# DuckTapeDevOps/kubernetes-cloud

Measured on AMD Instinct MI355X. Metric: GPT-J-6B finetune tokens/sec, higher is better.
Workload: dtype bf16; 1 GPU; model=gpt-j-6b, global_batch=32, micro_batch=16, grad_accum=2, seq_len=2048, parallelism=dp1, activation_checkpointing=False

## Files before the change

csrc/kernels/attention_tiled.hip:

```cpp
#include "common.h"

#include <type_traits>

namespace {

constexpr float kLog2e = 1.4426950408889634f;
constexpr float kLn2 = 0.6931471805599453f;
constexpr float kRescaleThr = 8.0f;

#ifdef KCA_ATTN_STAMPS
__device__ unsigned long long g_attn_stamps[64];
__device__ __forceinline__ unsigned long long ast_now() {
  unsigned long long t;
  __builtin_amdgcn_sched_barrier(0);
  asm volatile("s_memtime %0\n\ts_waitcnt lgkmcnt(0)" : "=s"(t)::"memory");
  __builtin_amdgcn_sched_barrier(0);
  return t;
}
#define ASTAMP_DECL                                            \
  unsigned long long st_acc_[8] = {0, 0, 0, 0, 0, 0, 0, 0}; \
  unsigned long long st_prev_ = ast_now();
#define ASTAMP(k)                           \
  do {                                      \
    const unsigned long long n_ = ast_now(); \
    st_acc_[k] += n_ - st_prev_;            \
    st_prev_ = n_;                          \
  } while (0)
#define ASTAMP_FLUSH(base)                                                          \
  do {                                                                              \
    st_acc_[7] = 1;                                                                 \
    if ((threadIdx.x & 63) == 0)                                                    \
      for (int i_ = 0; i_ < 8; ++i_) atomicAdd(&g_attn_stamps[(base) + i_], st_acc_[i_]); \
  } while (0)
#else
#define ASTAMP_DECL
#define ASTAMP(k) \
  do {            \
  } while (0)
#define ASTAMP_FLUSH(base) \
  do {                     \
  } while (0)
#endif


struct FastFwdParams {
  const bf16_t* q; const bf16_t* k; const bf16_t* v;
  bf16_t* o; float* lse;
  int* flags;
  long long q_sb, q_st, q_sh, k_sb, k_st, k_sh, v_sb, v_st, v_sh;
  long long o_sb, o_st, o_sh;
  int B, Sq, Sk, H, Hkv;
  float scale;
};

typedef __attribute__((address_space(3))) bf16x4 lds_bf16x4_t;
typedef unsigned int u32x4 __attribute__((ext_vector_type(4)));

__device__ __forceinline__ bf16x4 lds_tr4(const char* base, int byte_off) {
  return __builtin_amdgcn_ds_read_tr16_b64_v4bf16(
      (lds_bf16x4_t*)(reinterpret_cast<uintptr_t>(base + byte_off)));
}

__device__ __forceinline__ bf16x8 lds_b128(const char* base, int byte_off) {
  return *reinterpret_cast<const bf16x8*>(base + byte_off);
}

template <int D>
__device__ __forceinline__ int img_off(int row, int ch) {
  return (row >> 3) * 16 * D + 512 * (ch >> 2) + 64 * (row & 7) + 16 * ((ch & 3) ^ ((row >> 2) & 3));
}

__device__ __forceinline__ bf16x8 cat8(bf16x4 a, bf16x4 b) {
  return __builtin_shufflevector(a, b, 0, 1, 2, 3, 4, 5, 6, 7);
}

__device__ __forceinline__ uint32_t pk_bf16(float lo, float hi) {
  return pack_bf16x2(lo, hi);
}

__device__ __forceinline__ __amdgpu_buffer_rsrc_t head_rsrc(const bf16_t* b) {
  const unsigned long long a = (unsigned long long)b;
  const unsigned long long au = ((unsigned long long)__builtin_amdgcn_readfirstlane((unsigned)(a >> 32)) << 32) |
                                (unsigned)__builtin_amdgcn_readfirstlane((unsigned)a);
  return __builtin_amdgcn_make_buffer_rsrc((void*)au, (short)0, 0x7fffffff, 0x00020000);
}

template <int D, bool POW2 = (256 % (D / 8)) == 0>
struct Stager;

template <int D>
struct Stager<D, true> {
  static constexpr int NCH = D / 8, CPT = 32 * NCH / 256, RPI = 256 / NCH;
  long long ok_, ov_;
  int row0_, ch_;
  __amdgpu_buffer_rsrc_t rk_, rv_;
  int vok_[CPT], vov_[CPT];
  __device__ __forceinline__ Stager(int tid, long long k_st, long long v_st) {
    row0_ = tid / NCH;
    ch_ = tid % NCH;
    ok_ = (long long)row0_ * k_st + ch_ * 8;
    ov_ = (long long)row0_ * v_st + ch_ * 8;
  }
  __device__ __forceinline__ void bind(const bf16_t* kb, const bf16_t* vb, long long k_st, long long v_st) {
#pragma unroll
    for (int i = 0; i < CPT; ++i) {
      vok_[i] = (int)((ok_ + (long long)i * RPI * k_st) * 2);
      vov_[i] = (int)((ov_ + (long long)i * RPI * v_st) * 2);
    }
    set_base(kb, vb);
  }
  __device__ __forceinline__ void set_base(const bf16_t* kb, const bf16_t* vb) {
    rk_ = head_rsrc(kb);
    rv_ = head_rsrc(vb);
  }
  __device__ __forceinline__ void load(u32x4 (&sk)[CPT], u32x4 (&sv)[CPT], const bf16_t* kb, const bf16_t* vb,
                                       int k0, long long k_st, long long v_st) const {
    const int sok = __builtin_amdgcn_readfirstlane((int)(k0 * k_st * 2));
    const int sov = __builtin_amdgcn_readfirstlane((int)(k0 * v_st * 2));
#pragma unroll
    for (int i = 0; i < CPT; ++i) {
      const auto a = __builtin_amdgcn_raw_buffer_load_b128(rk_, vok_[i], sok, 0);
      const auto b = __builtin_amdgcn_raw_buffer_load_b128(rv_, vov_[i], sov, 0);
      sk[i] = *reinterpret_cast<const u32x4*>(&a);
      sv[i] = *reinterpret_cast<const u32x4*>(&b);
    }
  }
  __device__ __forceinline__ void store(const u32x4 (&sk)[CPT], const u32x4 (&sv)[CPT], char* buf) const {
#pragma unroll
    for (int i = 0; i < CPT; ++i) {
      const int o = img_off<D>(row0_ + i * RPI, ch_);
      *reinterpret_cast<u32x4*>(buf + o) = sk[i];
      *reinterpret_cast<u32x4*>(buf + 32 * D * 2 + o) = sv[i];
    }
  }
};

template <int D>
struct Stager<D, false> {
  static constexpr int NCH = D / 8, TOT = 32 * NCH, CPT = (TOT + 255) / 256;
  static_assert(D % 32 == 0 && TOT % 64 == 0, "tiled attention: D multiple of 32");
  long long ok_[CPT], ov_[CPT];
  int lds_[CPT];
  bool tail_;
  __device__ __forceinline__ Stager(int tid, long long k_st, long long v_st) {
#pragma unroll
    for (int i = 0; i < CPT; ++i) {
      const int idx = min(tid + 256 * i, TOT - 1);
      const int row = idx / NCH, ch = idx % NCH;
      ok_[i] = (long long)row * k_st + ch * 8;
      ov_[i] = (long long)row * v_st + ch * 8;
      lds_[i] = img_off<D>(row, ch);
    }
    tail_ = tid + 256 * (CPT - 1) < TOT;
  }
  __device__ __forceinline__ void bind(const bf16_t*, const bf16_t*, long long, long long) {}
  __device__ __forceinline__ void set_base(const bf16_t*, const bf16_t*) {}
  __device__ __forceinline__ void load(u32x4 (&sk)[CPT], u32x4 (&sv)[CPT], const bf16_t* kb, const bf16_t* vb,
                                       int k0, long long k_st, long long v_st) const {
    const bf16_t* kr = kb + (long long)k0 * k_st;
    const bf16_t* vr = vb + (long long)k0 * v_st;
#pragma unroll
    for (int i = 0; i < CPT; ++i) {
      sk[i] = *reinterpret_cast<const u32x4*>(kr + ok_[i]);
      sv[i] = *reinterpret_cast<const u32x4*>(vr + ov_[i]);
    }
  }
  __device__ __forceinline__ void store(const u32x4 (&sk)[CPT], const u32x4 (&sv)[CPT], char* buf) const {
#pragma unroll
    for (int i = 0; i < CPT; ++i) {
      if (i < CPT - 1 || tail_) {
        *reinterpret_cast<u32x4*>(buf + lds_[i]) = sk[i];
        *reinterpret_cast<u32x4*>(buf + 32 * D * 2 + lds_[i]) = sv[i];
      }
    }
  }
};

template <int D, int DS>
struct StagerNarrow {
  static constexpr int NCH = DS / 8, TOT = 32 * NCH, CPT = 1;
  static_assert(TOT <= 256 && TOT % 64 == 0, "narrow stager: one chunk per thread, whole waves");
  int vok_[1], vov_[1], lds_;
  bool on_;
  __amdgpu_buffer_rsrc_t rk_, rv_;
  __device__ __forceinline__ StagerNarrow(int tid, long long k_st, long long v_st) {
    const int idx = min(tid, TOT - 1), row = idx / NCH, ch = idx % NCH;
    vok_[0] = (int)(((long long)row * k_st + ch * 8) * 2);
    vov_[0] = (int)(((long long)row * v_st + ch * 8) * 2);
    lds_ = img_off<D>(row, ch);
    on_ = tid < TOT;
  }
  __device__ __forceinline__ void bind(const bf16_t* kb, const bf16_t* vb, long long, long long) { set_base(kb, vb); }
  __device__ __forceinline__ void set_base(const bf16_t* kb, const bf16_t* vb) {
    rk_ = head_rsrc(kb);
    rv_ = head_rsrc(vb);
  }
  __device__ __forceinline__ void load(u32x4 (&sk)[1], u32x4 (&sv)[1], const bf16_t*, const bf16_t*, int k0,
                                       long long k_st, long long v_st) const {
    const int sok = __builtin_amdgcn_readfirstlane((int)(k0 * k_st * 2));
    const int sov = __builtin_amdgcn_readfirstlane((int)(k0 * v_st * 2));
    const auto a = __builtin_amdgcn_raw_buffer_load_b128(rk_, vok_[0], sok, 0);
    const auto b = __builtin_amdgcn_raw_buffer_load_b128(rv_, vov_[0], sov, 0);
    sk[0] = *reinterpret_cast<const u32x4*>(&a);
    sv[0] = *reinterpret_cast<const u32x4*>(&b);
  }
  __device__ __forceinline__ void store(const u32x4 (&sk)[1], const u32x4 (&sv)[1], char* buf) const {
    if (on_) {
      *reinterpret_cast<u32x4*>(buf + lds_) = sk[0];
      *reinterpret_cast<u32x4*>(buf + 32 * D * 2 + lds_) = sv[0];
    }
  }
};

template <int D, int DS>
using StagerFor = std::conditional_t<DS == D, Stager<D>, StagerNarrow<D, DS>>;

template <int D, int DS = D>
__device__ __forceinline__ void store_tile_lds(bf16_t* row0, long long st, const f32x16 (&acc)[D / 32], int lane,
                                               float mul, char* lds) {
  constexpr int NCH = D / 8, RB = D * 2, NCS = DS / 8;
  const int l32 = lane & 31, hh = lane >> 5;
#pragma unroll
  for (int db = 0; db < D / 32; ++db) {
#pragma unroll
    for (int g = 0; g < 4; ++g) {
      uint2 w;
      w.x = pk_bf16(acc[db][4 * g] * mul, acc[db][4 * g + 1] * mul);
      w.y = pk_bf16(acc[db][4 * g + 2] * mul, acc[db][4 * g + 3] * mul);
      *reinterpret_cast<uint2*>(lds + l32 * RB + ((4 * db + g + l32) % NCH) * 16 + hh * 8) = w;
    }
  }
  asm volatile("" ::: "memory");
  static_assert((32 * NCS) % 64 == 0, "whole-wave epilogue rounds");
#pragma unroll
  for (int j = 0; j < 32 * NCS / 64; ++j) {
    const int idx = j * 64 + lane, r = idx / NCS, c = idx % NCS;
    const uint4 v = *reinterpret_cast<const uint4*>(lds + r * RB + ((c + r) % NCH) * 16);
    *reinterpret_cast<uint4*>(row0 + (long long)r * st + c * 8) = v;
  }
  asm volatile("" ::: "memory");
}

template <int D, bool CAUSAL, int OC = -1, int DS = D, int MC = -1>
__global__ void __launch_bounds__(256, (D <= 128 ? 2 : 1)) attn_fwd_tiled_kernel(FastFwdParams p) {
  constexpr int BM = 128, BN = 32;
  constexpr int TILE = BN * D * 2;
  constexpr int KS = DS / 16;
  using Stg = StagerFor<D, DS>;
  constexpr int CPT = Stg::CPT;
  __shared__ __attribute__((aligned(16))) char smem[3 * 2 * TILE];

  ASTAMP_DECL
  const int tid = threadIdx.x, lane = tid & 63, wave = tid >> 6;
  const int l32 = lane & 31, hh = lane >> 5, gi = lane & 15;
  const int nqb = p.Sq / BM;
  const int lid = xcd_remap(blockIdx.x, gridDim.x);
  const int qi = lid % nqb;
  const int qb = CAUSAL ? (nqb - 1 - qi) : qi;
  const int bh = lid / nqb;
  const int b = bh / p.H, h = bh % p.H;
  const int hk = h / (p.H / p.Hkv);
  const int off = p.Sk - p.Sq;
  const int q0 = qb * BM + wave * 32;
  const int qrow = q0 + l32;
  int kv_hi = p.Sk;
  if (CAUSAL) kv_hi = min(kv_hi, qb * BM + BM + off);
  const int ntiles = kv_hi > 0 ? (kv_hi + BN - 1) / BN : 0;
  static_assert(MC < 0 || (!CAUSAL && OC >= 0 && MC < DS), "max column: non-causal, with the row-sum column");
  const float sl2 = MC >= 0 ? 1.f : p.scale * kLog2e;

  const bf16_t* qp = p.q + b * p.q_sb + h * p.q_sh;
  const bf16_t* kp = p.k + b * p.k_sb + hk * p.k_sh;
  const bf16_t* vp = p.v + b * p.v_sb + hk * p.v_sh;

  bf16x8 qf[KS];
#pragma unroll
  for (int s = 0; s < KS; ++s)
    qf[s] = *reinterpret_cast<const bf16x8*>(qp + (long long)qrow * p.q_st + 16 * s + 8 * hh);

  f32x16 oacc[D / 32];
#pragma unroll
  for (int i = 0; i < D / 32; ++i)
#pragma unroll
    for (int r = 0; r < 16; ++r) oacc[i][r] = 0.f;
  float m = 0.f, lsum = 0.f;

  Stg stg(tid, p.k_st, p.v_st);
  stg.bind(kp, vp, p.k_st, p.v_st);
  u32x4 sk[CPT], sv[CPT];
  if constexpr (DS < D) {
    constexpr int PC = D / 8 - DS / 8, NZ = 3 * 32 * PC;
// ... 632 lines not shown
      const int img = i / (32 * PC), row = (i / PC) % 32, ch = NCS + i % PC;
      *reinterpret_cast<u32x4*>(smem + img * TILE + img_off<D>(row, ch)) = u32x4{0, 0, 0, 0};
    }
  }
  f32x16 dk[D / 32], dv[D / 32];
#pragma unroll
  for (int i = 0; i < D / 32; ++i)
#pragma unroll
    for (int r = 0; r < 16; ++r) { dk[i][r] = 0.f; dv[i][r] = 0.f; }

  int q_lo = 0;
  if (CAUSAL) q_lo = max(0, kb * BK - off) & ~(BQ - 1);
  const int nqt = (p.Sq - q_lo) / BQ;
  const int total = nqt * grp;

  Stg stg(tid, p.q_st, p.do_st);
  stg.bind(p.q + b * p.q_sb + hk * grp * p.q_sh, p.dout + b * p.do_sb + hk * grp * p.do_sh, p.q_st, p.do_st);
  u32x4 sq[CPT], sg[CPT];
  float lreg = 0.f;
  int be, bo, b1, b2;
  row_bases<D>(l32, hh, be, bo);
  tr_bases<D>(lane, b1, b2);

#define KCA_DKDV_LOAD(it_)                                                                     \
  {                                                                                            \
    const int hq_ = hk * grp + (it_) / nqt, qt_ = q_lo + ((it_) % nqt) * BQ;                   \
    if (grp > 1) stg.set_base(p.q + b * p.q_sb + hq_ * p.q_sh, p.dout + b * p.do_sb + hq_ * p.do_sh); \
    stg.load(sq, sg, p.q + b * p.q_sb + hq_ * p.q_sh, p.dout + b * p.do_sb + hq_ * p.do_sh, qt_,   \
             p.q_st, p.do_st);                                                                 \
    if (tid < 64) {                                                                            \
      const long long li_ = ((long long)b * p.H + hq_) * p.Sq + qt_ + (tid & 31);              \
      lreg = tid < 32 ? p.lse[li_] * kLog2e : p.delta[li_];                                    \
    }                                                                                          \
  }
#define KCA_DKDV_STORE(buf_)                                                                   \
  {                                                                                            \
    stg.store(sq, sg, smem + (buf_) * 2 * TILE);                                               \
    if (tid < 64) reinterpret_cast<float*>(smem + LOFF)[(buf_) * 64 + tid] = lreg;             \
  }

  if (total > 0) {
    KCA_DKDV_LOAD(0);
    KCA_DKDV_STORE(0);
  }
  __syncthreads();
  ASTAMP(0);
  auto tile_step = [&](int it, auto masked) {
    constexpr bool MASKED = decltype(masked)::value;
    const int qt = q_lo + (it % nqt) * BQ;
    const char* Qs = smem + (it & 1) * 2 * TILE;
    const char* Gs = Qs + TILE;
    const float* ls = reinterpret_cast<const float*>(smem + LOFF) + (it & 1) * 64;
    const int nx = min(it + 1, total - 1);
    KCA_DKDV_LOAD(nx);
    asm volatile("" ::: "memory");
    ASTAMP(1);
    f32x16 sacc, dpacc;
#pragma unroll
    for (int r = 0; r < 16; ++r) { sacc[r] = 0.f; dpacc[r] = 0.f; }
    {
      bf16x8 fq0 = row_frag<D>(Qs, be, bo, 0), fg0 = row_frag<D>(Gs, be, bo, 0), fv0 = row_frag<D>(vimg, be, bo, 0);
      bf16x8 fq1, fg1, fv1;
      __builtin_amdgcn_sched_group_barrier(0x100, 3, 0);
#pragma unroll
      for (int s = 0; s < KSD; ++s) {
        bf16x8& cq = (s & 1) ? fq1 : fq0;
        bf16x8& cg = (s & 1) ? fg1 : fg0;
        bf16x8& cv = (s & 1) ? fv1 : fv0;
        bf16x8& nq = (s & 1) ? fq0 : fq1;
        bf16x8& ng = (s & 1) ? fg0 : fg1;
        bf16x8& nv = (s & 1) ? fv0 : fv1;
        if (s + 1 < KSD) {
          nq = row_frag<D>(Qs, be, bo, s + 1);
          ng = row_frag<D>(Gs, be, bo, s + 1);
          nv = row_frag<D>(vimg, be, bo, s + 1);
          __builtin_amdgcn_sched_group_barrier(0x100, 3, 0);
        }
        sacc = __builtin_amdgcn_mfma_f32_32x32x16_bf16(cq, kf[s], sacc, 0, 0, 0);
        dpacc = __builtin_amdgcn_mfma_f32_32x32x16_bf16(cg, cv, dpacc, 0, 0, 0);
        __builtin_amdgcn_sched_group_barrier(0x8, 2, 0);
      }
    }
    ASTAMP(2);
    const int lim = key - qt - off - 4 * hh;
    bf16x8 p0, p1, s0, s1;
#pragma unroll
    for (int g = 0; g < 4; ++g) {
      const f32x4 lq = *reinterpret_cast<const f32x4*>(ls + 8 * g + 4 * hh);
      const f32x4 dq4 = *reinterpret_cast<const f32x4*>(ls + 32 + 8 * g + 4 * hh);
#pragma unroll
      for (int j = 0; j < 4; ++j) {
        const int r = 4 * g + j;
        float pr = __builtin_amdgcn_exp2f(fmaf(sacc[r], sl2, -lq[j]));
        if constexpr (MASKED) {
          if (8 * g + j < lim) pr = 0.f;
        }
        const float ds = pr * (dpacc[r] - dq4[j]);
        if (r < 8) { p0[r] = (__bf16)pr; s0[r] = (__bf16)ds; }
        else { p1[r - 8] = (__bf16)pr; s1[r - 8] = (__bf16)ds; }
      }
    }
    ASTAMP(3);
    {
      bf16x8 a0 = tr_frag<D>(Gs, b1, b2, 0, 0), a1 = tr_frag<D>(Gs, b1, b2, 1, 0);
      bf16x8 a2 = tr_frag<D>(Qs, b1, b2, 0, 0), a3 = tr_frag<D>(Qs, b1, b2, 1, 0);
      bf16x8 n0, n1, n2, n3;
      __builtin_amdgcn_sched_group_barrier(0x100, 8, 0);
#pragma unroll
      for (int db = 0; db < D / 32; ++db) {
        bf16x8& c0 = (db & 1) ? n0 : a0;
        bf16x8& c1 = (db & 1) ? n1 : a1;
        bf16x8& c2 = (db & 1) ? n2 : a2;
        bf16x8& c3 = (db & 1) ? n3 : a3;
        bf16x8& x0 = (db & 1) ? a0 : n0;
        bf16x8& x1 = (db & 1) ? a1 : n1;
        bf16x8& x2 = (db & 1) ? a2 : n2;
        bf16x8& x3 = (db & 1) ? a3 : n3;
        if (db + 1 < D / 32) {
          x0 = tr_frag<D>(Gs, b1, b2, 0, db + 1);
          x1 = tr_frag<D>(Gs, b1, b2, 1, db + 1);
          x2 = tr_frag<D>(Qs, b1, b2, 0, db + 1);
          x3 = tr_frag<D>(Qs, b1, b2, 1, db + 1);
          __builtin_amdgcn_sched_group_barrier(0x100, 8, 0);
        }
        dv[db] = __builtin_amdgcn_mfma_f32_32x32x16_bf16(c0, p0, dv[db], 0, 0, 0);
        dv[db] = __builtin_amdgcn_mfma_f32_32x32x16_bf16(c1, p1, dv[db], 0, 0, 0);
        dk[db] = __builtin_amdgcn_mfma_f32_32x32x16_bf16(c2, s0, dk[db], 0, 0, 0);
        dk[db] = __builtin_amdgcn_mfma_f32_32x32x16_bf16(c3, s1, dk[db], 0, 0, 0);
        __builtin_amdgcn_sched_group_barrier(0x8, 4, 0);
      }
    }
    ASTAMP(4);
    asm volatile("" ::: "memory");
    if (it + 1 < total) KCA_DKDV_STORE((it + 1) & 1);
    __syncthreads();
    ASTAMP(5);
  };
  for (int it = 0; it < total; ++it) tile_step(it, std::integral_constant<bool, CAUSAL>{});
#undef KCA_DKDV_LOAD
#undef KCA_DKDV_STORE
  if constexpr (D == 96) {
    store_acc_t<D>(p.dk + b * p.dk_sb + hk * p.dk_sh + (long long)key * p.dk_st, dk, hh, p.scale);
    store_acc_t<D>(p.dv + b * p.dv_sb + hk * p.dv_sh + (long long)key * p.dv_st, dv, hh, 1.f);
  } else {
    store_tile_lds<D, DS>(p.dk + b * p.dk_sb + hk * p.dk_sh + (long long)kw * p.dk_st, p.dk_st, dk, lane, p.scale,
                      smem + wave * 32 * D * 2);
    store_tile_lds<D, DS>(p.dv + b * p.dv_sb + hk * p.dv_sh + (long long)kw * p.dv_st, p.dv_st, dv, lane, 1.f,
                      smem + wave * 32 * D * 2);
  }
  ASTAMP(6);
  ASTAMP_FLUSH(32);
}

inline bool offsets_fit(long long rows, long long stride) { return (rows + 128) * stride * 2 < (1ll << 31); }

}

static int g_attn_variant = 1;
KCA_API int kca_attn_set_variant(int v) {
  g_attn_variant = v;
  return 0;
}

KCA_API int kca_attn_fwd_tiled(const void* q, const void* k, const void* v, void* o, float* lse,
                               long long q_sb, long long q_st, long long q_sh, long long k_sb,
                               long long k_st, long long k_sh, long long v_sb, long long v_st,
                               long long v_sh, long long o_sb, long long o_st, long long o_sh,
                               int B, int Sq, int Sk, int H, int Hkv, int d, int causal,
                               float scale, int rowsum_col, int max_col, int* flags, hipStream_t stream) {
  if ((d != 48 && d != 64 && d != 96 && d != 128 && d != 160 && d != 256) || Sq % 128 || Sk % 32 || Sq <= 0 ||
      H % Hkv || !flags)
    return 1;
  if (max_col >= 0 && (max_col != 40 || rowsum_col != 40 || d != 48)) return 1;
  if (d == 48 && causal) return 1;
  if (rowsum_col >= 0 && (rowsum_col != 40 || (d != 64 && d != 48) || causal)) return 1;
  if (causal && Sk < Sq) return 1;
  if (!offsets_fit(Sk, k_st) || !offsets_fit(Sk, v_st)) return 1;
  FastFwdParams p{(const bf16_t*)q, (const bf16_t*)k, (const bf16_t*)v, (bf16_t*)o, lse, flags,
                  q_sb, q_st, q_sh, k_sb, k_st, k_sh, v_sb, v_st, v_sh, o_sb, o_st, o_sh,
                  B, Sq, Sk, H, Hkv, scale};
  dim3 grid((Sq / 128) * B * H);
  (void)hipGetLastError();
  if (d == 256 && (g_attn_variant & 1) && Sq % 256 == 0) {
    dim3 g8((Sq / 256) * B * H);
    if (causal) hipLaunchKernelGGL((attn_fwd_w8_kernel<256, true>), g8, dim3(512), 0, stream, p);
    else hipLaunchKernelGGL((attn_fwd_w8_kernel<256, false>), g8, dim3(512), 0, stream, p);
  } else if (d == 256) {
    if (causal) hipLaunchKernelGGL((attn_fwd_tiled_kernel<256, true>), grid, dim3(256), 0, stream, p);
    else hipLaunchKernelGGL((attn_fwd_tiled_kernel<256, false>), grid, dim3(256), 0, stream, p);
  } else if (d == 160) {
    if (causal) hipLaunchKernelGGL((attn_fwd_tiled_kernel<160, true>), grid, dim3(256), 0, stream, p);
    else hipLaunchKernelGGL((attn_fwd_tiled_kernel<160, false>), grid, dim3(256), 0, stream, p);
  } else if (d == 128) {
    if (causal) hipLaunchKernelGGL((attn_fwd_tiled_kernel<128, true>), grid, dim3(256), 0, stream, p);
    else hipLaunchKernelGGL((attn_fwd_tiled_kernel<128, false>), grid, dim3(256), 0, stream, p);
  } else if (d == 96) {
    if (causal) hipLaunchKernelGGL((attn_fwd_tiled_kernel<96, true>), grid, dim3(256), 0, stream, p);
    else hipLaunchKernelGGL((attn_fwd_tiled_kernel<96, false>), grid, dim3(256), 0, stream, p);
  } else if (d == 48) {
    if (max_col == 40) hipLaunchKernelGGL((attn_fwd_tiled_kernel<64, false, 40, 48, 40>), grid, dim3(256), 0, stream, p);
    else if (rowsum_col == 40) hipLaunchKernelGGL((attn_fwd_tiled_kernel<64, false, 40, 48>), grid, dim3(256), 0, stream, p);
    else hipLaunchKernelGGL((attn_fwd_tiled_kernel<64, false, -1, 48>), grid, dim3(256), 0, stream, p);
  } else {
    if (causal) hipLaunchKernelGGL((attn_fwd_tiled_kernel<64, true>), grid, dim3(256), 0, stream, p);
    else if (rowsum_col == 40) hipLaunchKernelGGL((attn_fwd_tiled_kernel<64, false, 40>), grid, dim3(256), 0, stream, p);
    else hipLaunchKernelGGL((attn_fwd_tiled_kernel<64, false>), grid, dim3(256), 0, stream, p);
  }
  return hipGetLastError() == hipSuccess ? 0 : 3;
}

KCA_API int kca_attn_fwd_wide(const void* q, const void* k, const void* v, void* o, float* lse, long long q_sb,
                              long long q_st, long long q_sh, long long k_sb, long long k_st, long long k_sh,
                              long long v_sb, long long v_st, long long v_sh, long long o_sb, long long o_st,
                              long long o_sh, int B, int Sq, int Sk, int H, int Hkv, int d, float scale, int* flags,
                              hipStream_t stream) {
  if (d != 512 || Sq % 128 || Sk % 32 || Sq <= 0 || Sk <= 0 || H % Hkv || !flags) return 1;
  if (!offsets_fit(Sk, k_st) || !offsets_fit(Sk, v_st)) return 1;
  if ((q_st | k_st | v_st | o_st) % 8) return 1;
  FastFwdParams p{(const bf16_t*)q, (const bf16_t*)k, (const bf16_t*)v, (bf16_t*)o, lse, flags,
                  q_sb, q_st, q_sh, k_sb, k_st, k_sh, v_sb, v_st, v_sh, o_sb, o_st, o_sh,
                  B, Sq, Sk, H, Hkv, scale};
  (void)hipGetLastError();
  hipLaunchKernelGGL((attn_fwd_w8_kernel<512, false, 4, 2>), dim3((Sq / 128) * B * H), dim3(256), 0, stream, p);
  return hipGetLastError() == hipSuccess ? 0 : 3;
}

KCA_API int kca_attn_bwd_tiled(const void* q, const void* k, const void* v, const void* dout,
                               void* dq, void* dk, void* dv, const float* lse, const float* delta,
                               long long q_sb, long long q_st, long long q_sh, long long k_sb,
                               long long k_st, long long k_sh, long long v_sb, long long v_st,
                               long long v_sh, long long do_sb, long long do_st, long long do_sh,
                               long long dq_sb, long long dq_st, long long dq_sh, long long dk_sb,
                               long long dk_st, long long dk_sh, long long dv_sb, long long dv_st,
                               long long dv_sh, int B, int Sq, int Sk, int H, int Hkv, int d,
                               int causal, float scale, hipStream_t stream) {
  if ((d != 48 && d != 64 && d != 96 && d != 128 && d != 160 && d != 256) || Sq % 128 || Sk % 128 || Sq <= 0 ||
      H % Hkv)
    return 1;
  if (d == 48 && causal) return 1;
  if (causal && Sk < Sq) return 1;
  if (!offsets_fit(Sk, k_st) || !offsets_fit(Sk, v_st) || !offsets_fit(Sq, q_st) || !offsets_fit(Sq, do_st)) return 1;
  FastBwdParams p{(const bf16_t*)q, (const bf16_t*)k, (const bf16_t*)v, (const bf16_t*)dout,
                  (bf16_t*)dq, (bf16_t*)dk, (bf16_t*)dv, lse, delta,
                  q_sb, q_st, q_sh, k_sb, k_st, k_sh, v_sb, v_st, v_sh, do_sb, do_st, do_sh,
                  dq_sb, dq_st, dq_sh, dk_sb, dk_st, dk_sh, dv_sb, dv_st, dv_sh,
                  B, Sq, Sk, H, Hkv, scale};
  dim3 g1((Sk / 128) * B * Hkv), g2((Sq / 128) * B * H);
  if (d == 48) {
    hipLaunchKernelGGL((attn_bwd_dkdv_tiled_kernel<64, false, 48>), g1, dim3(256), 0, stream, p);
    hipLaunchKernelGGL((attn_bwd_dq_tiled_kernel<64, false, 48>), g2, dim3(256), 0, stream, p);
  } else if (d == 256) {
    if (causal) {
      hipLaunchKernelGGL((attn_bwd_dkdv_tiled_kernel<256, true>), g1, dim3(256), 0, stream, p);
      hipLaunchKernelGGL((attn_bwd_dq_tiled_kernel<256, true>), g2, dim3(256), 0, stream, p);
    } else {
      hipLaunchKernelGGL((attn_bwd_dkdv_tiled_kernel<256, false>), g1, dim3(256), 0, stream, p);
      hipLaunchKernelGGL((attn_bwd_dq_tiled_kernel<256, false>), g2, dim3(256), 0, stream, p);
    }
  } else if (d == 160) {
    if (causal) {
      hipLaunchKernelGGL((attn_bwd_dkdv_tiled_kernel<160, true>), g1, dim3(256), 0, stream, p);
      hipLaunchKernelGGL((attn_bwd_dq_tiled_kernel<160, true>), g2, dim3(256), 0, stream, p);
    } else {
      hipLaunchKernelGGL((attn_bwd_dkdv_tiled_kernel<160, false>), g1, dim3(256), 0, stream, p);
      hipLaunchKernelGGL((attn_bwd_dq_tiled_kernel<160, false>), g2, dim3(256), 0, stream, p);
    }
  } else if (d == 96) {
    if (causal) {
      hipLaunchKernelGGL((attn_bwd_dkdv_tiled_kernel<96, true>), g1, dim3(256), 0, stream, p);
      hipLaunchKernelGGL((attn_bwd_dq_tiled_kernel<96, true>), g2, dim3(256), 0, stream, p);
    } else {
      hipLaunchKernelGGL((attn_bwd_dkdv_tiled_kernel<96, false>), g1, dim3(256), 0, stream, p);
      hipLaunchKernelGGL((attn_bwd_dq_tiled_kernel<96, false>), g2, dim3(256), 0, stream, p);
    }
  } else if (d == 128) {
    if (causal) {
      hipLaunchKernelGGL((attn_bwd_dkdv_tiled_kernel<128, true>), g1, dim3(256), 0, stream, p);
      hipLaunchKernelGGL((attn_bwd_dq_tiled_kernel<128, true>), g2, dim3(256), 0, stream, p);
    } else {
      hipLaunchKernelGGL((attn_bwd_dkdv_tiled_kernel<128, false>), g1, dim3(256), 0, stream, p);
      hipLaunchKernelGGL((attn_bwd_dq_tiled_kernel<128, false>), g2, dim3(256), 0, stream, p);
    }
  } else {
    if (causal) {
      hipLaunchKernelGGL((attn_bwd_dkdv_tiled_kernel<64, true>), g1, dim3(256), 0, stream, p);
      hipLaunchKernelGGL((attn_bwd_dq_tiled_kernel<64, true>), g2, dim3(256), 0, stream, p);
    } else {
      hipLaunchKernelGGL((attn_bwd_dkdv_tiled_kernel<64, false>), g1, dim3(256), 0, stream, p);
      hipLaunchKernelGGL((attn_bwd_dq_tiled_kernel<64, false>), g2, dim3(256), 0, stream, p);
    }
  }
  return 0;
}

#ifdef KCA_ATTN_STAMPS
KCA_API int kca_attn_stamps(unsigned long long* host, int reset) {
  if (hipMemcpyFromSymbol(host, HIP_SYMBOL(g_attn_stamps), sizeof(unsigned long long) * 64) != hipSuccess) return 1;
  if (reset) {
    unsigned long long z[64] = {0};
    if (hipMemcpyToSymbol(HIP_SYMBOL(g_attn_stamps), z, sizeof(z)) != hipSuccess) return 1;
  }
  return 0;
}
#endif
```

kubernetes_cloud_amd/ops/_lib.py:

```python
from __future__ import annotations

import ctypes
import os
import threading

import torch

_HERE = os.path.dirname(os.path.abspath(__file__))
LIB_DIR = os.path.join(os.path.dirname(_HERE), "_lib")
DEBUG = os.environ.get("KCA_DEBUG", "0") in ("1", "true")
KERNEL_LIB = os.path.join(LIB_DIR, "libkca_kernels_debug.so" if DEBUG else "libkca_kernels.so")
KERNEL_LIB = os.environ.get("KCA_KERNEL_LIB") or KERNEL_LIB

_lock = threading.Lock()
_lib = None
_err: str | None = None

P = ctypes.c_void_p
I = ctypes.c_int
LL = ctypes.c_longlong
F = ctypes.c_float

_SIGS = {
    "kca_layernorm_fwd": [P, P, P, P, P, P, P, P, P, I, I, F, P],
    "kca_gemm_lt": [P, LL, P, LL, P, P, LL, P, LL, I, I, I, F, P, LL, P],
    "kca_gemm_lt_gelu": [P, LL, P, LL, I, P, P, LL, P, LL, I, I, I, P, LL, P],
    "kca_layernorm_bwd_parts": [I],
    "kca_layernorm_bwd": [P, P, P, P, P, P, P, P, P, I, P, I, I, P],
    "kca_gelu_fwd": [P, P, LL, I, P],
    "kca_gelu_fwd_f16": [P, P, LL, I, P],
    "kca_gelu_bwd": [P, P, P, LL, I, P],
    "kca_quick_gelu_fwd": [P, P, LL, P],
    "kca_quick_gelu_bwd": [P, P, P, LL, P],
    "kca_geglu_fwd": [P, P, LL, I, P],
    "kca_add_bias_nhwc": [P, P, P, P, LL, I, P],
    "kca_add_bias2_nhwc": [P, P, P, P, P, LL, I, P],
    "kca_colsum_bf16": [P, P, I, I, I, P],
    "kca_geglu_bwd": [P, P, P, LL, I, P],
    "kca_rope": [P, P, I, I, LL, I, LL, LL, LL, LL, I, I, P, P, P, F, P],
    "kca_accum_grad": [P, P, F, I, LL, P],
    "kca_accum_grad_pair": [P, P, P, F, LL, P],
    "kca_accum_grad_multi": [P, I, F, P],
    "kca_cast_f32_bf16": [P, P, LL, P],
    "kca_ema": [P, P, F, LL, P],
    "kca_cross_entropy_fwd": [P, LL, P, I, I, I, P, P, P],
    "kca_cross_entropy_bwd": [P, LL, P, P, P, F, I, I, I, P, LL, P],
    "kca_adamw": [P, P, P, P, P, LL, P, F, F, F, F, F, F, F, P, P, P],
    "kca_sumsq": [P, LL, P, P, P],
    "kca_adamw8bit": [P, P, P, P, P, P, P, LL, P, F, F, F, F, F, F, F, P, P, P],
    "kca_clip_coef": [P, F, F, P, P, P, P],
    "kca_attn_fwd": [P] * 5 + [LL] * 12 + [I] * 7 + [F, P, P, I, P, I, I, P, P],
    "kca_attn_bwd_preprocess": [P, P, P, LL, LL, LL, LL, LL, LL, I, I, I, I, P],
    "kca_attn_bwd": [P] * 10 + [LL] * 21 + [I] * 7 + [F, P, P, I, P, P],
    "kca_attn_fwd_wide": [P] * 5 + [LL] * 12 + [I] * 6 + [F, P, P],
    "kca_attn_set_tiled": [I],
    "kca_attn_set_variant": [I],
    "kca_transpose_bf16": [P, LL, P, LL, I, I, P],
    "kca_gelu_fwd_t": [P, LL, P, LL, P, LL, I, I, I, P],
    "kca_gelu_bwd_t": [P, LL, P, LL, P, LL, P, LL, P, I, I, I, P],
    "kca_transpose_colsum": [P, LL, P, LL, P, I, I, P],
    "kca_col_reduce_f32": [P, I, I, P, P, P],
    "kca_accum_grad_2d": [P, P, LL, I, I, F, I, P],
    "kca_groupnorm_fwd": [P, P, P, P, P, P, P, I, I, I, I, F, I, P],
    "kca_groupnorm_bwd": [P, P, P, P, P, P, P, P, P, P, I, I, I, I, I, P],
    "kca_groupnorm_nhwc_ws": [I, I, I],
    "kca_groupnorm_nhwc_fwd": [P, P, P, P, P, P, P, I, I, I, I, F, I, P],
    "kca_groupnorm_nhwc_fwd_add": [P, P, P, P, LL, P, P, P, P, I, I, I, I, F, I, P],
    "kca_groupnorm_nhwc_cat_fwd": [P, P, P, P, P, P, P, P, P, P, I, I, I, I, I, I, F, I, P],
    "kca_groupnorm_nhwc_bwd": [P, P, P, P, P, P, P, P, P, P, I, I, I, I, I, P],
    "kca_skinny_set_smallk": [I],
    "kca_conv3x3_fwd": [P, P, P, P, I, I, I, I, I, P],
    "kca_conv3x3_set_variant": [I],
    "kca_conv3x3_wflip": [P, P, I, I, P],
    "kca_conv3x3_wgrad_splits": [I, I, I, I, I],
    "kca_conv3x3_wgrad": [P, P, P, P, I, I, I, I, I, I, P],
    "kca_skinny_gemm": [P, LL, P, P, P, LL, I, I, I, I, P],
    "kca_skinny_set_splitk": [I],
    "kca_mm_skinny_set": [I],
    "kca_ln_skinny_gemm": [P, LL, P, P, P, LL, P, P, F, P, P, P, LL, I, I, I, I, P, P],
    "kca_ln_rows": [P, LL, P, P, P, LL, P, P, F, P, I, I, P],
    "kca_embed_ln_rows": [P, LL, P, P, P, I, P, LL, P, P, F, P, I, I, P],
    "kca_decode_prep": [P, LL, I, I, I, I, I, I, P, P, P, P, P, P, LL, LL, LL, P, I, I, P],
    "kca_decode_chunk": [I, I, I],
    "kca_decode_set_stamps": [P],
    "kca_decode_attn": [P, LL, P, P, LL, LL, LL, P, P, P, LL, P, LL, I, I, I, I, I, I, F, P, P, I, I, I, P],
    "kca_sd_noise_prep": [P, P, P, P, P, P, P, P, P, I, I, I, I, F, I, ctypes.c_ulonglong, LL, I, P],
    "kca_mse_split_fwd": [P, P, LL, LL, F, P, I, P, P],
    "kca_mse_split_bwd": [P, P, P, LL, LL, F, P, P],
    "kca_sd_lms_step": [P, P, P, P, LL, P, I, I, I, I, I, F, F, F, P],
    "kca_decode_prep_attn": [P, LL, P, P, LL, LL, LL, P, P, P, LL, P, LL, I, I, I, I, I, I, F, P, P, I, I, I, I, P,
                             P, I, I, P],
    "kca_im2col2x2_nhwc": [P, P, I, I, I, I, P],
    "kca_phase_to_dense_nhwc": [P, P, P, I, I, I, I, P],
    "kca_upsample2x_nhwc": [P, P, I, I, I, I, P],
    "kca_dense_to_phase_nhwc": [P, P, I, I, I, I, P],
    "kca_col2im2x2_nhwc": [P, P, I, I, I, I, P],
    "kca_pad_br_nhwc": [P, P, I, I, I, I, P],
    "kca_gemv_dual_ln": [P, P, I, P, P, I, P, P, P, P, P, P, P, F, P, P, P, P, I, P],
    "kca_sample_logits": [P, LL, I, I, I, P, P, P, P, P, P, P, I, P, LL, P, P, P, P, P, I, P],
}


_SIGS["kca_decode_prep_attn_gemv"] = _SIGS["kca_decode_prep_attn"][:-2] + [P, P, P, P, I, I, I, I, P]

for _n in ("kca_decode_prep_attn", "kca_ln_rows", "kca_embed_ln_rows", "kca_decode_prep_attn_gemv",
           "kca_gemv_dual_ln", "kca_skinny_gemm"):
    _SIGS[_n + "_f16"] = _SIGS[_n]


def _load():
    global _lib, _err
    if _lib is not None or _err is not None:
        return _lib
    with _lock:
        if _lib is not None or _err is not None:
            return _lib
        if not os.path.exists(KERNEL_LIB):
            _err = f"{KERNEL_LIB} not built (run `python tools/build_ext.py`)"
            return None
        try:
            lib = ctypes.CDLL(KERNEL_LIB, mode=ctypes.RTLD_GLOBAL)
        except OSError as e:
            _err = f"failed to load {KERNEL_LIB}: {e}"
            return None
        for name, argtypes in _SIGS.items():
            fn = getattr(lib, name, None)
            if fn is None:
                continue
            fn.argtypes = argtypes
            fn.restype = ctypes.c_int
        _lib = lib
        return _lib


def available() -> bool:
    return _load() is not None


def require():
    lib = _load()
    if lib is None:
        raise RuntimeError(
            "kubernetes_cloud_amd native kernels unavailable: " + str(_err)
            + " -- refusing to fall back to eager PyTorch on a GPU tensor")
    return lib


def has(name: str) -> bool:
    lib = _load()
    return lib is not None and hasattr(lib, name)


SYNC_LAUNCH = os.environ.get("KCA_SYNC_LAUNCH", "0") in ("1", "true")


LAUNCHES = [0]


def call(name: str, *args):
    lib = require()
    fn = getattr(lib, name)
    LAUNCHES[0] += 1
    rc = fn(*args)
    if rc != 0:
        raise RuntimeError(f"{name} returned status {rc} (unsupported shape/arguments)")
    if SYNC_LAUNCH and torch.cuda.is_available():
        try:
            torch.cuda.synchronize()
        except RuntimeError as e:
            raise RuntimeError(f"GPU fault after native launch {name}: {e}") from e
    return rc


def call_rc(name: str, *args) -> int:
    rc = getattr(require(), name)(*args)
    LAUNCHES[0] += rc == 0
    if rc == 0 and SYNC_LAUNCH and torch.cuda.is_available():
        torch.cuda.synchronize()
    return rc


def stream() -> int:
    return torch.cuda.current_stream().cuda_stream


def ptr(t: torch.Tensor | None) -> int | None:
    return None if t is None else t.data_ptr()


def native_f16(*tensors: torch.Tensor | None) -> bool:
    on_gpu = False
    for t in tensors:
        if t is not None and t.is_cuda:
            on_gpu = True
            if t.dtype != torch.float16:
                return False
    return on_gpu


def use_native(*tensors: torch.Tensor | None) -> bool:
    on_gpu = False
    for t in tensors:
        if t is not None and t.is_cuda:
            on_gpu = True
            if t.dtype != torch.bfloat16:
                return False
    return on_gpu
```

kubernetes_cloud_amd/ops/attention.py:

```python
from __future__ import annotations

import math

import torch

from . import _lib
from .rope import apply_rotary_


def attention_reference(q, k, v, causal: bool, scale: float | None = None,
                        kv_len: torch.Tensor | None = None, alibi: torch.Tensor | None = None,
                        window: int = 0):
    B, Sq, H, D = q.shape
    Sk, Hkv = k.shape[1], k.shape[2]
    scale = scale if scale is not None else 1.0 / math.sqrt(D)
    qf = q.float().transpose(1, 2)
    kf = k.float().transpose(1, 2)
    vf = v.float().transpose(1, 2)
    if Hkv != H:
        rep = H // Hkv
        kf = kf.repeat_interleave(rep, dim=1)
        vf = vf.repeat_interleave(rep, dim=1)
    s = torch.matmul(qf, kf.transpose(-1, -2)) * scale
    qi = torch.arange(Sq, device=q.device)[:, None]
    ki = torch.arange(Sk, device=q.device)[None, :]
    off = Sk - Sq
    if alibi is not None:
        s = s + alibi.float().view(1, H, 1, 1) * (ki - qi - off).float()
    mask = torch.zeros(B, 1, Sq, Sk, dtype=torch.bool, device=q.device)
    if causal:
        mask = mask | (ki > qi + off)
    if window:
        mask = mask | (ki <= qi + off - window)
    if kv_len is not None and kv_len.dtype == torch.bool:
        mask = mask | ~kv_len.to(q.device).view(B, 1, 1, Sk)
    elif kv_len is not None:
        mask = mask | (ki[None, None] >= kv_len.view(B, 1, 1, 1).to(q.device))
    s = s.masked_fill(mask, float("-inf"))
    lse = torch.logsumexp(s, dim=-1)
    p = torch.exp(s - lse[..., None])
    p = torch.nan_to_num(p, nan=0.0)
    o = torch.matmul(p, vf).transpose(1, 2)
    return o.to(q.dtype), lse


def set_tiled_path(enable: bool) -> None:
    _lib.call("kca_attn_set_tiled", int(bool(enable)))


_VARIANT = [1]


def set_variant(v: int) -> int:
    _lib.call("kca_attn_set_variant", int(v))
    old, _VARIANT[0] = _VARIANT[0], int(v)
    return old


def _strides(t):
    return t.stride(0), t.stride(1), t.stride(2)


def pack_key_mask(mask: torch.Tensor) -> torch.Tensor:
    B, Sk = mask.shape
    W = (Sk + 31) // 32
    m = torch.zeros(B, W * 32, dtype=torch.int64, device=mask.device)
    m[:, :Sk] = mask.to(torch.int64)
    words = (m.view(B, W, 32) << torch.arange(32, device=mask.device, dtype=torch.int64)).sum(-1)
    words = torch.where(words >= 2 ** 31, words - 2 ** 32, words)
    return words.to(torch.int32).contiguous()


def _masks(kv_len):
    if kv_len is None:
        return None, None
    return (kv_len, None) if kv_len.dim() == 1 else (None, kv_len)


def _fwd(q, k, v, causal, scale, kv_len, alibi, out=None, window: int = 0, rowsum_col: int = -1,
         max_col: int = -1):
    B, Sq, H, D = q.shape
    Sk, Hkv = k.shape[1], k.shape[2]
    o = out if out is not None else torch.empty(B, Sq, H, D, device=q.device, dtype=q.dtype)
    lse = torch.empty(B, H, Sq, device=q.device, dtype=torch.float32)
    flags = torch.empty(4 * ((Sq + 127) // 128) * B * H, device=q.device, dtype=torch.int32)
    lens, km = _masks(kv_len)
    _lib.call("kca_attn_fwd", q.data_ptr(), k.data_ptr(), v.data_ptr(), o.data_ptr(), lse.data_ptr(),
              *_strides(q), *_strides(k), *_strides(v), *_strides(o),
              B, Sq, Sk, H, Hkv, D, int(causal), float(scale), _lib.ptr(alibi), _lib.ptr(lens),
              int(window), _lib.ptr(km), int(rowsum_col), int(max_col), flags.data_ptr(), _lib.stream())
    return o, lse


def _bwd(q, k, v, o, do, lse, dq, dk, dv, causal, scale, kv_len, alibi, window: int = 0):
    B, Sq, H, D = q.shape
    Sk, Hkv = k.shape[1], k.shape[2]
    delta = torch.empty(B, H, Sq, device=q.device, dtype=torch.float32)
    _lib.call("kca_attn_bwd_preprocess", o.data_ptr(), do.data_ptr(), delta.data_ptr(),
              *_strides(o), *_strides(do), B, Sq, H, D, _lib.stream())
    _lib.call("kca_attn_bwd", q.data_ptr(), k.data_ptr(), v.data_ptr(), o.data_ptr(), do.data_ptr(),
              dq.data_ptr(), dk.data_ptr(), dv.data_ptr(), lse.data_ptr(), delta.data_ptr(),
              *_strides(q), *_strides(k), *_strides(v), *_strides(do),
              *_strides(dq), *_strides(dk), *_strides(dv),
              B, Sq, Sk, H, Hkv, D, int(causal), float(scale), _lib.ptr(alibi), _lib.ptr(_masks(kv_len)[0]),
              int(window), _lib.ptr(_masks(kv_len)[1]), _lib.stream())


def _check(q, k, v):
    for t in (q, k, v):
        if t.dim() != 4 or t.stride(-1) != 1:
            raise ValueError("attention expects [B, S, H, D] views with unit last stride")
        if t.dtype != torch.bfloat16:
            raise ValueError("native attention is bf16")
    D = q.shape[-1]
    if D % 8 or D > 256:
        raise ValueError(f"head_dim {D} unsupported (multiple of 8, <= 256)")


class _FlashAttnFn(torch.autograd.Function):
    @staticmethod
    def forward(ctx, q, k, v, causal, scale, kv_len, alibi, window):
        _check(q, k, v)
        o, lse = _fwd(q, k, v, causal, scale, kv_len, alibi, window=window)
        ctx.save_for_backward(q, k, v, o, lse, kv_len, alibi)
        ctx.causal, ctx.scale, ctx.window = causal, scale, window
        return o

    @staticmethod
    def backward(ctx, do):
        q, k, v, o, lse, kv_len, alibi = ctx.saved_tensors
        do = do.contiguous()
        dq = torch.empty(q.shape, device=q.device, dtype=q.dtype)
        dk = torch.empty(k.shape, device=k.device, dtype=k.dtype)
        dv = torch.empty(v.shape, device=v.device, dtype=v.dtype)
        _bwd(q, k, v, o, do, lse, dq, dk, dv, ctx.causal, ctx.scale, kv_len, alibi, ctx.window)
        return dq, dk, dv, None, None, None, None, None


def native_mask(kv_len, device):
    if kv_len is None:
        return None
    if kv_len.dtype == torch.bool:
        return pack_key_mask(kv_len.to(device))
    return kv_len.to(device=device, dtype=torch.int32).contiguous()


def flash_attention(q: torch.Tensor, k: torch.Tensor, v: torch.Tensor, causal: bool = False,
                    scale: float | None = None, kv_len: torch.Tensor | None = None,
                    alibi: torch.Tensor | None = None, window: int = 0, rowsum_col: int = -1,
                    max_col: int = -1) -> torch.Tensor:
    scale = scale if scale is not None else 1.0 / math.sqrt(q.shape[-1])
    if alibi is not None:
        alibi = alibi.to(device=q.device, dtype=torch.float32).contiguous()
    if rowsum_col >= 0 and _lib.use_native(q, k, v) and not torch.is_grad_enabled():
        _check(q, k, v)
        return _fwd(q, k, v, causal, scale, native_mask(kv_len, q.device), alibi, window=window,
                    rowsum_col=rowsum_col, max_col=max_col)[0]
    if max_col >= 0:
        raise ValueError("max_col needs rowsum_col and the native inference path")
    if _lib.use_native(q, k, v):
        return _FlashAttnFn.apply(q, k, v, causal, scale, native_mask(kv_len, q.device), alibi, int(window))
    o, _ = attention_reference(q, k, v, causal, scale, kv_len, alibi, window)
    return o


def wide_head_attention(q: torch.Tensor, k: torch.Tensor, v: torch.Tensor, scale: float):
    if not (_lib.use_native(q, k, v) and q.dim() == 3 and q.shape[-1] == 512 and not torch.is_grad_enabled()):
        return None
    if any(t.stride(-1) != 1 or t.dtype != torch.bfloat16 for t in (q, k, v)):
        return None
    B, Sq, D = q.shape
    Sk = k.shape[1]
    if Sq % 128 or Sk % 32:
        return None
    o = torch.empty(B, Sq, D, device=q.device, dtype=q.dtype)
    flags = torch.empty(4 * (Sq // 128) * B, device=q.device, dtype=torch.int32)
    st = lambda t: (t.stride(0), t.stride(1), 0)
    rc = _lib.call_rc("kca_attn_fwd_wide", q.data_ptr(), k.data_ptr(), v.data_ptr(), o.data_ptr(), None,
                      *st(q), *st(k), *st(v), *st(o), B, Sq, Sk, 1, 1, D, float(scale), flags.data_ptr(),
                      _lib.stream())
    if rc != 0 or bool(flags.any()):
        return None
    return o


class _QKVRopeAttnFn(torch.autograd.Function):

    @staticmethod
    def forward(ctx, qkv, H, D, rot, interleaved, base, causal, scale, kv_len):
        B, S, _ = qkv.shape
        v5 = qkv.view(B, S, 3, H, D)
        q, k, v = v5[:, :, 0], v5[:, :, 1], v5[:, :, 2]
        if rot > 0:
            apply_rotary_(q, k, rot, S, interleaved, base, 1.0)
        o, lse = _fwd(q, k, v, causal, scale, kv_len, None)
        ctx.save_for_backward(qkv, o, lse, kv_len)
        ctx.cfg = (H, D, rot, interleaved, base, causal, scale)
        return o.view(B, S, H * D)

    @staticmethod
    def backward(ctx, do):
        qkv, o, lse, kv_len = ctx.saved_tensors
        H, D, rot, interleaved, base, causal, scale = ctx.cfg
# ... 40 lines not shown
```

Baseline: 34560 tokens/s.

## Add 8-wave split dK/dV backward kernel for head dim 256

Adds a 512-thread dK/dV backward kernel for D=256. Four waves compute P and dV while the other four compute dP, dS and dK, and they exchange P through shared memory with triple-buffered Q/dO tiles. The Stager is generalised to 512 threads. The default variant becomes 3 so this path is used for non-GQA D=256, which is GPT-J's head dim. The split is meant to raise per-block parallelism and overlap the two gradient chains, at the cost of more LDS, one block per CU, and added synchronisation.

```diff
diff --git a/csrc/kernels/attention_tiled.hip b/csrc/kernels/attention_tiled.hip
--- a/csrc/kernels/attention_tiled.hip
+++ b/csrc/kernels/attention_tiled.hip
@@ -85,12 +85,13 @@
   return __builtin_amdgcn_make_buffer_rsrc((void*)au, (short)0, 0x7fffffff, 0x00020000);
 }
 
-template <int D, bool POW2 = (256 % (D / 8)) == 0>
+template <int D, bool POW2 = (256 % (D / 8)) == 0, int NT = 256>
 struct Stager;
 
-template <int D>
-struct Stager<D, true> {
-  static constexpr int NCH = D / 8, CPT = 32 * NCH / 256, RPI = 256 / NCH;
+template <int D, int NT>
+struct Stager<D, true, NT> {
+  static constexpr int NCH = D / 8, CPT = 32 * NCH / NT, RPI = NT / NCH;
+  static_assert(CPT >= 1 && NT % NCH == 0, "stager: at least one chunk per thread");
   long long ok_, ov_;
   int row0_, ch_;
   __amdgpu_buffer_rsrc_t rk_, rv_;
@@ -119,16 +120,26 @@
     const int sov = __builtin_amdgcn_readfirstlane((int)(k0 * v_st * 2));
 #pragma unroll
     for (int i = 0; i < CPT; ++i) {
-      const auto a = __builtin_amdgcn_raw_buffer_load_b128(rk_, vok_[i], sok, 0);
-      const auto b = __builtin_amdgcn_raw_buffer_load_b128(rv_, vov_[i], sov, 0);
-      sk[i] = *reinterpret_cast<const u32x4*>(&a);
-      sv[i] = *reinterpret_cast<const u32x4*>(&b);
+      if constexpr (NT == 256) {
+        const auto a = __builtin_amdgcn_raw_buffer_load_b128(rk_, vok_[i], sok, 0);
+        const auto b = __builtin_amdgcn_raw_buffer_load_b128(rv_, vov_[i], sov, 0);
+        sk[i] = *reinterpret_cast<const u32x4*>(&a);
+        sv[i] = *reinterpret_cast<const u32x4*>(&b);
+      } else {
+        const int sk_i = __builtin_amdgcn_readfirstlane((int)((k0 + i * RPI) * k_st * 2));
+        const int sv_i = __builtin_amdgcn_readfirstlane((int)((k0 + i * RPI) * v_st * 2));
+        const auto a = __builtin_amdgcn_raw_buffer_load_b128(rk_, vok_[0], sk_i, 0);
+        const auto b = __builtin_amdgcn_raw_buffer_load_b128(rv_, vov_[0], sv_i, 0);
+        sk[i] = *reinterpret_cast<const u32x4*>(&a);
+        sv[i] = *reinterpret_cast<const u32x4*>(&b);
+      }
     }
   }
   __device__ __forceinline__ void store(const u32x4 (&sk)[CPT], const u32x4 (&sv)[CPT], char* buf) const {
 #pragma unroll
     for (int i = 0; i < CPT; ++i) {
-      const int o = img_off<D>(row0_ + i * RPI, ch_);
+      const int o = (NT != 256 && RPI % 16 == 0) ? img_off<D>(row0_, ch_) + i * (RPI / 8) * 16 * D
+                                                : img_off<D>(row0_ + i * RPI, ch_);
       *reinterpret_cast<u32x4*>(buf + o) = sk[i];
       *reinterpret_cast<u32x4*>(buf + 32 * D * 2 + o) = sv[i];
     }
@@ -136,7 +147,7 @@
 };
 
 template <int D>
-struct Stager<D, false> {
+struct Stager<D, false, 256> {
   static constexpr int NCH = D / 8, TOT = 32 * NCH, CPT = (TOT + 255) / 256;
   static_assert(D % 32 == 0 && TOT % 64 == 0, "tiled attention: D multiple of 32");
   long long ok_[CPT], ov_[CPT];
@@ -1075,11 +1086,253 @@
   ASTAMP_FLUSH(32);
 }
 
+template <int D, bool CAUSAL>
+__global__ void __launch_bounds__(512, 1) attn_bwd_dkdv_w8_kernel(FastBwdParams p) {
+  constexpr int BK = 128, BQ = 32;
+  constexpr int TILE = BQ * D * 2;
+  using Stg = Stager<D, true, 512>;
+  constexpr int CPT = Stg::CPT, KSD = D / 16;
+  constexpr int PSZ = 4 * 64 * 16;
+  constexpr int POFF = 3 * 2 * TILE;
+  constexpr int LOFF = POFF + 2 * 4 * PSZ;
+  __shared__ __attribute__((aligned(16))) char smem[LOFF + 3 * 64 * 4];
+  static_assert(8 * 32 * D * 2 <= LOFF, "epilogue images of the 8 waves");
+  ASTAMP_DECL
+
+  const int tid = threadIdx.x, lane = tid & 63;
+  const int wave = __builtin_amdgcn_readfirstlane(tid >> 6);
+  const int pw = wave & 3;
+  const bool kside = wave < 4;
+  const int l32 = lane & 31, hh = lane >> 5;
+  const int nkb = p.Sk / BK;
+  const int lid = xcd_remap(blockIdx.x, gridDim.x);
+  const int kb = lid % nkb, bh = lid / nkb;
+  const int b = bh / p.H, h = bh % p.H;
+  const int off = p.Sk - p.Sq;
+  const int kw = kb * BK + pw * 32;
+  const int key = kw + l32;
+  const float sl2 = p.scale * kLog2e;
+
+  bf16x8 rf[KSD];
+  {
+    const bf16_t* rp = kside ? p.v + b * p.v_sb + h * p.v_sh + (long long)key * p.v_st
+                             : p.k + b * p.k_sb + h * p.k_sh + (long long)key * p.k_st;
+#pragma unroll
+    for (int s = 0; s < KSD; ++s) rf[s] = *reinterpret_cast<const bf16x8*>(rp + 16 * s + 8 * hh);
+  }
+  f32x16 acc[D / 32];
+#pragma unroll
+  for (int i = 0; i < D / 32; ++i)
+#pragma unroll
+    for (int r = 0; r < 16; ++r) acc[i][r] = 0.f;
+
+  int q_lo = 0;
+  if (CAUSAL) q_lo = max(0, kb * BK - off) & ~(BQ - 1);
+  const int total = (p.Sq - q_lo) / BQ;
+
+  const bf16_t* qb = p.q + b * p.q_sb + h * p.q_sh;
+  const bf16_t* gb = p.dout + b * p.do_sb + h * p.do_sh;
+  Stg stg(tid, p.q_st, p.do_st);
+  stg.bind(qb, gb, p.q_st, p.do_st);
+  u32x4 sq[CPT], sg[CPT];
+  float lreg = 0.f;
+  int be, bo, b1, b2;
+  row_bases<D>(l32, hh, be, bo);
+  tr_bases<D>(lane, b1, b2);
+
+  const float* lsrc = (kside ? p.delta : p.lse) + ((long long)b * p.H + h) * p.Sq + q_lo;
+  const float lmul = kside ? 1.f : kLog2e;
+  const bool lwave = pw == 0 && lane < 32;
+  auto load_tile = [&](int it) {
+    stg.load(sq, sg, qb, gb, q_lo + it * BQ, p.q_st, p.do_st);
+    if (lwave) lreg = lsrc[it * BQ + lane];
+  };
+  auto store_tile = [&](int buf) {
+    stg.store(sq, sg, smem + buf * 2 * TILE);
+    if (lwave) reinterpret_cast<float*>(smem + LOFF)[buf * 64 + (kside ? 32 : 0) + lane] = lreg * lmul;
+  };
+
+  if (total > 0) {
+    load_tile(0);
+    store_tile(0);
+  }
+  __syncthreads();
+  ASTAMP(0);
+
+  if (!kside) {
+    __builtin_amdgcn_s_setprio(1);
+    auto v_step = [&](int t, int cur, int nxt) {
+      const char* Qs = smem + cur * 2 * TILE;
+      const char* Gs = Qs + TILE;
+      const float* ls = reinterpret_cast<const float*>(smem + LOFF) + cur * 64;
+      float* pb = reinterpret_cast<float*>(smem + POFF + ((t & 1) * 4 + pw) * PSZ);
+      const int qt = q_lo + t * BQ;
+      load_tile(min(t + 1, total - 1));
+      asm volatile("" ::: "memory");
+      ASTAMP(1);
+      f32x16 sacc;
+#pragma unroll
+      for (int r = 0; r < 16; ++r) sacc[r] = 0.f;
+      {
+        constexpr int PF = 1;
+        bf16x8 f[PF + 1];
+#pragma unroll
+        for (int s = 0; s < PF; ++s) f[s] = row_frag<D>(Qs, be, bo, s);
+        __builtin_amdgcn_sched_group_barrier(0x100, PF, 0);
+#pragma unroll
+        for (int s = 0; s < KSD; ++s) {
+          if (s + PF < KSD) {
+            f[(s + PF) % (PF + 1)] = row_frag<D>(Qs, be, bo, s + PF);
+            __builtin_amdgcn_sched_group_barrier(0x100, 1, 0);
+          }
+          sacc = __builtin_amdgcn_mfma_f32_32x32x16_bf16(f[s % (PF + 1)], rf[s], sacc, 0, 0, 0);
+          __builtin_amdgcn_sched_group_barrier(0x8, 1, 0);
+        }
+      }
+      ASTAMP(2);
+      const int lim = key - qt - off - 4 * hh;
+      bf16x8 p0, p1;
+#pragma unroll
+      for (int g = 0; g < 4; ++g) {
+        const f32x4 lq = *reinterpret_cast<const f32x4*>(ls + 8 * g + 4 * hh);
+        f32x4 pg;
+#pragma unroll
+        for (int j = 0; j < 4; ++j) {
+          const int r = 4 * g + j;
+          float pr = __builtin_amdgcn_exp2f(fmaf(sacc[r], sl2, -lq[j]));
+          if constexpr (CAUSAL) {
+            if (8 * g + j < lim) pr = 0.f;
+          }
+          pg[j] = pr;
+          if (r < 8) p0[r] = (__bf16)pr;
+          else p1[r - 8] = (__bf16)pr;
+        }
+        *reinterpret_cast<f32x4*>(pb + (g * 64 + lane) * 4) = pg;
+      }
+      ASTAMP(3);
+      {
+        bf16x8 f[3];
+        f[0] = tr_frag<D>(Gs, b1, b2, 0, 0);
+        f[1] = tr_frag<D>(Gs, b1, b2, 1, 0);
+        __builtin_amdgcn_sched_group_barrier(0x100, 4, 0);
+#pragma unroll
+        for (int i = 0; i < D / 16; ++i) {
+          if (i + 2 < D / 16) {
+            f[(i + 2) % 3] = tr_frag<D>(Gs, b1, b2, i & 1, (i + 2) >> 1);
+            __builtin_amdgcn_sched_group_barrier(0x100, 2, 0);
+          }
+          acc[i >> 1] = __builtin_amdgcn_mfma_f32_32x32x16_bf16(f[i % 3], (i & 1) ? p1 : p0, acc[i >> 1], 0, 0, 0);
+          __builtin_amdgcn_sched_group_barrier(0x8, 1, 0);
+        }
+      }
+      ASTAMP(4);
+      asm volatile("" ::: "memory");
+      if (t + 1 < total) store_tile(nxt);
+      __syncthreads();
+      ASTAMP(5);
+    };
+    int cur = 0;
+    for (int t = 0; t < total; ++t) {
+      const int nxt = cur == 2 ? 0 : cur + 1;
+      v_step(t, cur, nxt);
+      cur = nxt;
+    }
+    __syncthreads();
+  } else {
+    auto k_step = [&](int t, int cur, int nxt) {
+      const char* Qs = smem + cur * 2 * TILE;
+      const char* Gs = Qs + TILE;
+      const float* ls = reinterpret_cast<const float*>(smem + LOFF) + cur * 64 + 32;
+      const float* pb = reinterpret_cast<const float*>(smem + POFF + ((t & 1) * 4 + pw) * PSZ);
+      ASTAMP(1);
+      f32x16 dpacc;
+#pragma unroll
+      for (int r = 0; r < 16; ++r) dpacc[r] = 0.f;
+      {
+        constexpr int PF = 1;
+        bf16x8 f[PF + 1];
+#pragma unroll
+        for (int s = 0; s < PF; ++s) f[s] = row_frag<D>(Gs, be, bo, s);
+        __builtin_amdgcn_sched_group_barrier(0x100, PF, 0);
+#pragma unroll
+        for (int s = 0; s < KSD; ++s) {
+          if (s + PF < KSD) {
+            f[(s + PF) % (PF + 1)] = row_frag<D>(Gs, be, bo, s + PF);
+            __builtin_amdgcn_sched_group_barrier(0x100, 1, 0);
+          }
+          dpacc = __builtin_amdgcn_mfma_f32_32x32x16_bf16(f[s % (PF + 1)], rf[s], dpacc, 0, 0, 0);
+          __builtin_amdgcn_sched_group_barrier(0x8, 1, 0);
+        }
+      }
+      ASTAMP(2);
+      load_tile(min(t + 2, total - 1));
+      asm volatile("" ::: "memory");
+      bf16x8 s0, s1;
+#pragma unroll
+      for (int g = 0; g < 4; ++g) {
+        const f32x4 pg = *reinterpret_cast<const f32x4*>(pb + (g * 64 + lane) * 4);
+        const f32x4 dq4 = *reinterpret_cast<const f32x4*>(ls + 8 * g + 4 * hh);
+#pragma unroll
+        for (int j = 0; j < 4; ++j) {
+          const int r = 4 * g + j;
+          const float ds = pg[j] * (dpacc[r] - dq4[j]);
+          if (r < 8) s0[r] = (__bf16)ds;
+          else s1[r - 8] = (__bf16)ds;
+        }
+      }
+      ASTAMP(3);
+      {
+        bf16x8 f[3];
+        f[0] = tr_frag<D>(Qs, b1, b2, 0, 0);
+        f[1] = tr_frag<D>(Qs, b1, b2, 1, 0);
+        __builtin_amdgcn_sched_group_barrier(0x100, 4, 0);
+#pragma unroll
+        for (int i = 0; i < D / 16; ++i) {
+          if (i + 2 < D / 16) {
+            f[(i + 2) % 3] = tr_frag<D>(Qs, b1, b2, i & 1, (i + 2) >> 1);
+            __builtin_amdgcn_sched_group_barrier(0x100, 2, 0);
+          }
+          acc[i >> 1] = __builtin_amdgcn_mfma_f32_32x32x16_bf16(f[i % 3], (i & 1) ? s1 : s0, acc[i >> 1], 0, 0, 0);
+          __builtin_amdgcn_sched_group_barrier(0x8, 1, 0);
+        }
+      }
+      ASTAMP(4);
+      asm volatile("" ::: "memory");
+      if (t + 2 < total) store_tile(nxt);
+      __syncthreads();
+      ASTAMP(5);
+    };
+    if (total > 1) {
+      load_tile(1);
+      store_tile(1);
+    }
+    __syncthreads();
+    int cur = 0;
+    for (int t = 0; t < total; ++t) {
+      const int nxt = cur == 0 ? 2 : cur - 1;
+      k_step(t, cur, nxt);
+      cur = cur == 2 ? 0 : cur + 1;
+    }
+  }
+  __builtin_amdgcn_s_setprio(0);
+  {
+    bf16_t* dst = kside ? p.dk + b * p.dk_sb + h * p.dk_sh + (long long)kw * p.dk_st
+                        : p.dv + b * p.dv_sb + h * p.dv_sh + (long long)kw * p.dv_st;
+    store_tile_lds<D>(dst, kside ? p.dk_st : p.dv_st, acc, lane, kside ? p.scale : 1.f, smem + wave * 32 * D * 2);
+  }
+  ASTAMP(6);
+  if (!kside) {
+    ASTAMP_FLUSH(40);
+  } else {
+    ASTAMP_FLUSH(56);
+  }
+}
+
 inline bool offsets_fit(long long rows, long long stride) { return (rows + 128) * stride * 2 < (1ll << 31); }
 
 }
 
-static int g_attn_variant = 1;
+static int g_attn_variant = 3;
 KCA_API int kca_attn_set_variant(int v) {
   g_attn_variant = v;
   return 0;
@@ -1173,11 +1426,14 @@
     hipLaunchKernelGGL((attn_bwd_dkdv_tiled_kernel<64, false, 48>), g1, dim3(256), 0, stream, p);
     hipLaunchKernelGGL((attn_bwd_dq_tiled_kernel<64, false, 48>), g2, dim3(256), 0, stream, p);
   } else if (d == 256) {
+    const bool w8 = (g_attn_variant & 2) && H == Hkv;
     if (causal) {
-      hipLaunchKernelGGL((attn_bwd_dkdv_tiled_kernel<256, true>), g1, dim3(256), 0, stream, p);
+      if (w8) hipLaunchKernelGGL((attn_bwd_dkdv_w8_kernel<256, true>), g1, dim3(512), 0, stream, p);
+      else hipLaunchKernelGGL((attn_bwd_dkdv_tiled_kernel<256, true>), g1, dim3(256), 0, stream, p);
       hipLaunchKernelGGL((attn_bwd_dq_tiled_kernel<256, true>), g2, dim3(256), 0, stream, p);
     } else {
-      hipLaunchKernelGGL((attn_bwd_dkdv_tiled_kernel<256, false>), g1, dim3(256), 0, stream, p);
+      if (w8) hipLaunchKernelGGL((attn_bwd_dkdv_w8_kernel<256, false>), g1, dim3(512), 0, stream, p);
+      else hipLaunchKernelGGL((attn_bwd_dkdv_tiled_kernel<256, false>), g1, dim3(256), 0, stream, p);
       hipLaunchKernelGGL((attn_bwd_dq_tiled_kernel<256, false>), g2, dim3(256), 0, stream, p);
     }
   } else if (d == 160) {
diff --git a/kubernetes_cloud_amd/ops/_lib.py b/kubernetes_cloud_amd/ops/_lib.py
--- a/kubernetes_cloud_amd/ops/_lib.py
+++ b/kubernetes_cloud_amd/ops/_lib.py
@@ -11,6 +11,7 @@
 DEBUG = os.environ.get("KCA_DEBUG", "0") in ("1", "true")
 KERNEL_LIB = os.path.join(LIB_DIR, "libkca_kernels_debug.so" if DEBUG else "libkca_kernels.so")
 KERNEL_LIB = os.environ.get("KCA_KERNEL_LIB") or KERNEL_LIB
+ATTN_VARIANT_ENV = os.environ.get("KCA_ATTN_VARIANT")
 
 _lock = threading.Lock()
 _lib = None
@@ -129,6 +130,8 @@
                 continue
             fn.argtypes = argtypes
             fn.restype = ctypes.c_int
+        if ATTN_VARIANT_ENV is not None and hasattr(lib, "kca_attn_set_variant"):
+            lib.kca_attn_set_variant(int(ATTN_VARIANT_ENV))
         _lib = lib
         return _lib
 
diff --git a/kubernetes_cloud_amd/ops/attention.py b/kubernetes_cloud_amd/ops/attention.py
--- a/kubernetes_cloud_amd/ops/attention.py
+++ b/kubernetes_cloud_amd/ops/attention.py
@@ -48,7 +48,8 @@
     _lib.call("kca_attn_set_tiled", int(bool(enable)))
 
 
-_VARIANT = [1]
+DEFAULT_VARIANT = 3
+_VARIANT = [int(_lib.ATTN_VARIANT_ENV) if _lib.ATTN_VARIANT_ENV is not None else DEFAULT_VARIANT]
 
 
 def set_variant(v: int) -> int:
```

Measured after the change: 34940 tokens/s (median of 6 runs). 1.01x the previous value.
